# keichi/sdn-mpi-router

Measured on AMD Instinct MI355X. Metric: all-pairs routes/sec + % HBM roofline, k=48 fat-tree, 1/2/4/8 MI355X, higher is better.
Workload: dtype int32; 1 GPU; fat_tree:48 all-pairs dfs route tables (find_route); fabric=fat_tree:48, V=2880, E=110592, table_layout=packed, endpoints=host-bearing switches (host pairs), parallelism=sources sharded over 1 GPU(s), steps_in_flight=1

## Files before the change

### include/sdnroute.h

```cpp
#ifndef SDNROUTE_H
#define SDNROUTE_H

#include <stdint.h>

#ifdef __cplusplus
extern "C" {
#endif

#define SDNR_ABI_VERSION 1

#define SDNR_OK          0
#define SDNR_ERR_INVAL (-22)
#define SDNR_ERR_NOMEM (-12)
#define SDNR_ERR_NODEV (-19)
#define SDNR_ERR_STATE (-77)
#define SDNR_ERR_HIP   (-5)

#define SDNR_DEVICE_PTRS 0x1u
#define SDNR_TIMING      0x2u
#define SDNR_SAME_TABLES 0x4u
#define SDNR_LOADS_TO_ROOT 0x8u
#define SDNR_LOADS_SPLIT_HOP 0x10u
#define SDNR_LFA_LINK_ONLY 0x20u

// ... 139 lines not shown
                         double *level, int32_t max_rounds, double *used,
                         int32_t *nrounds , uint32_t flags);

int sdnr_edge_ports(sdnr_ctx *ctx, const uint64_t *ends, int32_t nends,
                    const uint64_t *ports, int32_t nports, uint8_t *is_edge,
                    uint32_t flags);

int sdnr_last_kernel_ms(sdnr_ctx *ctx, float *ms);

int sdnr_last_launches(const sdnr_ctx *ctx, int32_t *launches);

int sdnr_last_dfs_searched(sdnr_ctx *ctx, int32_t *n);

int sdnr_last_dfs_form(const sdnr_ctx *ctx, int32_t *form);

int sdnr_last_sweeps(const sdnr_ctx *ctx, int32_t *sweeps);

const char *sdnr_last_kernel(const sdnr_ctx *ctx);

#ifdef __cplusplus
}
#endif

#endif
```

### sdn-mpi-router_amd/csrc/capi.hip

```cpp
#include <stdarg.h>
#include <stdio.h>
#include <stdlib.h>
#include <string.h>

#include <algorithm>
#include <array>
#include <map>
#include <string>
#include <thread>
#include <vector>

#include "common.h"

static thread_local char g_err[512] = "";

int sdnr_fail(int code, const char *fmt, ...)
{
    va_list ap;
    va_start(ap, fmt);
    vsnprintf(g_err, sizeof g_err, fmt, ap);
    va_end(ap);
    return code;
}

// ... 142 lines not shown
    if (c->twin_rep) (void)hipFree(c->twin_rep);
    c->twin_rep = nullptr;
    c->has_twins = false;
    ++c->upload_gen;
    memset(c->live_ring, 0, sizeof c->live_ring);
    if (c->radj16 && c->radj_owned) (void)hipFree(c->radj16);
    if (c->runs) (void)hipFree(c->runs);
    c->runs = nullptr;
    c->runs_R = 0;
    if (c->adjb) (void)hipFree(c->adjb);
    if (c->adjp) (void)hipFree(c->adjp);
    if (c->radjx) (void)hipFree(c->radjx);
    c->adjb = nullptr;
    c->adjp = nullptr;
    c->radjx = nullptr;
    if (c->adj16) (void)hipFree(c->adj16);
    if (c->deg32) (void)hipFree(c->deg32);
    if (c->radjw) (void)hipFree(c->radjw);
    c->radjw = nullptr;
    if (c->radjc) (void)hipFree(c->radjc);
    c->radjc = nullptr;
    if (c->dict_bp) (void)hipFree(c->dict_bp);
    if (c->dict_bt) (void)hipFree(c->dict_bt);
    if (c->dict_off) (void)hipFree(c->dict_off);
    c->dict_bp = nullptr;
    c->dict_bt = nullptr;
    c->dict_off = nullptr;
    c->dict_P = 0;
    c->dict_NB = 0;
    c->dict_bpw = 0;
// ... 276 lines not shown
    int rc;
    if ((rc = upload(reinterpret_cast<int32_t **>(&ctx->dict_bp), bp.data(), bp.size() * 4, 0,
                     ctx->stream)) ||
        (rc = upload(reinterpret_cast<int32_t **>(&ctx->dict_bt), bt.data(), bt.size() * 4, 0,
                     ctx->stream)) ||
        (rc = upload(&ctx->dict_off, off.data(), off.size() * 4, 0, ctx->stream)))
        return rc;
    SDNR_HIP(hipStreamSynchronize(ctx->stream));
    ctx->dict_P = (int32_t)tuples.size();
    ctx->dict_NB = (int32_t)blocks.size();
    ctx->dict_bpw = bpw;
    return SDNR_OK;
}

static int upload_twins(sdnr_ctx *ctx, int32_t V, int32_t E, const int32_t *row_ptr,
                        const int32_t *col)
{
    if (V == 0) return SDNR_OK;
    std::vector<int32_t> in_ptr((size_t)V + 1, 0), in_col((size_t)E);
    for (int32_t e = 0; e < E; ++e) in_ptr[(size_t)col[e] + 1]++;
    for (int32_t v = 0; v < V; ++v) in_ptr[(size_t)v + 1] += in_ptr[v];
    {
        std::vector<int32_t> fill(in_ptr.begin(), in_ptr.end() - 1);
        for (int32_t u = 0; u < V; ++u)
            for (int32_t e = row_ptr[u]; e < row_ptr[u + 1]; ++e) in_col[fill[col[e]]++] = u;
    }
    std::vector<uint64_t> hash((size_t)V);
    std::vector<int32_t> rep((size_t)V), order;
    auto mix = [](uint64_t h, uint64_t x) {
        h ^= x + 0x9E3779B97F4A7C15ull + (h << 6) + (h >> 2);
        return h * 0xFF51AFD7ED558CCDull;
// ... 26 lines not shown
            for (size_t k = i; k < j; ++k) {
                const int32_t r = order[k];
                if (rep[r] == r && same(row_ptr, col, r, v) &&
                    same(in_ptr.data(), in_col.data(), r, v)) {
                    rep[v] = r;
                    any = true;
                    break;
                }
            }
        }
    }
    int rc = upload(&ctx->twin_rep, rep.data(), sizeof(int32_t) * (size_t)V, 0, ctx->stream);
    if (rc) return rc;
    SDNR_HIP(hipStreamSynchronize(ctx->stream));
    ctx->has_twins = any;
    return SDNR_OK;
}

int sdnr_graph_upload(sdnr_ctx *ctx, int32_t V, int32_t E, const int32_t *row_ptr,
                      const int32_t *col, const int32_t *port)
{
    CHECK_CTX(ctx);
    int rc = graph_upload_one(ctx, V, E, row_ptr, col, port);
    for (int k = 0; k < ctx->npeers && !rc; ++k)
        rc = graph_upload_one(ctx->peers[k], V, E, row_ptr, col, port);
    if (rc) return rc;
    SDNR_HIP(hipSetDevice(ctx->device));
    return SDNR_OK;
}

// ... 22 lines not shown
            if (e > a && col[e] <= col[e - 1])
                return sdnr_fail(SDNR_ERR_INVAL,
                                 "graph_upload: row %d not strictly ascending at %d", u, e);
        }
    }
    SDNR_HIP(hipSetDevice(ctx->device));
    SDNR_HIP(hipStreamSynchronize(ctx->stream));
    free_graph(ctx);
    int rc;
    if ((rc = upload(&ctx->row_ptr, row_ptr, sizeof(int32_t) * ((size_t)V + 1), 0, ctx->stream)) ||
        (rc = upload(&ctx->col, col, sizeof(int32_t) * (size_t)E, kPad, ctx->stream)) ||
        (rc = upload(&ctx->port, port, sizeof(int32_t) * (size_t)E, kPad, ctx->stream))) {
        free_graph(ctx);
        return rc;
    }
    if ((rc = upload_twins(ctx, V, E, row_ptr, col))) {
        free_graph(ctx);
        return rc;
    }
    int32_t W = 0;
    if (maxdeg > 0 && maxdeg <= SDNR_WAVE && (size_t)V * maxdeg <= 2 * (size_t)E + 64)
        W = maxdeg;
    if (const char *f = getenv("SDNROUTE_ELL"))
        if (!strcmp(f, "0")) W = 0;
    if (W > 0) {
        std::vector<int32_t> ec((size_t)V * W, -1), ep((size_t)V * W, -1);
        for (int32_t u = 0; u < V; ++u)
            for (int32_t e = row_ptr[u]; e < row_ptr[u + 1]; ++e) {
                ec[(size_t)u * W + (e - row_ptr[u])] = col[e];
                ep[(size_t)u * W + (e - row_ptr[u])] = port[e];
            }
// ... 22 lines not shown
                                        hipMemcpyHostToDevice, ctx->stream);
            }
            if (he == hipSuccess) he = hipStreamSynchronize(ctx->stream);
            if (he != hipSuccess) {
                free_graph(ctx);
                return sdnr_hip_fail(he, "graph_upload(ell16)");
            }
        }
        SDNR_HIP(hipStreamSynchronize(ctx->stream));
        if ((rc = upload_dict(ctx, V, W, row_ptr, col))) {
            free_graph(ctx);
            return rc;
        }
    }
    int32_t max_indeg = 0x7FFFFFFF;
    if (V < 65535 && maxdeg <= SDNR_WAVE) {
        const size_t rows = ((size_t)V + 1) * SDNR_WAVE;
        std::vector<uint16_t> a16(rows, (uint16_t)V), r16(rows, (uint16_t)V);
        std::vector<int32_t> indeg((size_t)V + 1, 0);
        std::vector<uint32_t> d32(((size_t)V + 2) & ~(size_t)1, 0u);
        for (int32_t u = 0; u < V; ++u) {
            const int32_t d = row_ptr[u + 1] - row_ptr[u];
            d32[(size_t)u] = (uint32_t)d;
            for (int32_t e = row_ptr[u]; e < row_ptr[u + 1]; ++e) {
                a16[(size_t)u * SDNR_WAVE + (e - row_ptr[u])] = (uint16_t)col[e];
                indeg[col[e]]++;
            }
        }
        int32_t maxin = 0;
        for (int32_t v = 0; v < V; ++v) maxin = indeg[v] > maxin ? indeg[v] : maxin;
        max_indeg = maxin;
        bool sym = true;
        if (maxin <= SDNR_WAVE) {
            std::vector<int32_t> fill((size_t)V, 0);
            for (int32_t u = 0; u < V; ++u)
                for (int32_t e = row_ptr[u]; e < row_ptr[u + 1]; ++e) {
                    const int32_t v = col[e];
                    r16[(size_t)v * SDNR_WAVE + fill[v]++] = (uint16_t)u;
                }
            sym = a16 == r16;
        }
        hipError_t he = hipMalloc(reinterpret_cast<void **>(&ctx->adj16), rows * 2);
        if (he == hipSuccess)
            he = hipMemcpyAsync(ctx->adj16, a16.data(), rows * 2, hipMemcpyHostToDevice, ctx->stream);
        if (he == hipSuccess && maxin <= SDNR_WAVE) {
            he = hipMalloc(reinterpret_cast<void **>(&ctx->deg32), d32.size() * 4);
            if (he == hipSuccess)
                he = hipMemcpyAsync(ctx->deg32, d32.data(), d32.size() * 4, hipMemcpyHostToDevice,
                                    ctx->stream);
            if (he == hipSuccess && sym) {
                ctx->radj16 = ctx->adj16;
            } else if (he == hipSuccess) {
                he = hipMalloc(reinterpret_cast<void **>(&ctx->radj16), rows * 2);
                ctx->radj_owned = he == hipSuccess;
                if (he == hipSuccess)
                    he = hipMemcpyAsync(ctx->radj16, r16.data(), rows * 2, hipMemcpyHostToDevice,
                                        ctx->stream);
            }
        }
        const size_t dummy = (((size_t)V + 1 + 31) & ~(size_t)31);
        if (he == hipSuccess && maxin <= SDNR_WAVE && dummy + SDNR_WAVE <= 0xFFFF) {
            std::vector<uint16_t> w16(r16.size());
            const std::vector<uint16_t> &src16 = sym ? a16 : r16;
            const bool pair = maxin <= SDNR_WAVE / 2;
            const char *pe = sdnr_tune_env("SDNROUTE_DFS_PAIR");
            ctx->radj_pair = pair && !(pe && !strcmp(pe, "0"));
            auto at = [&](size_t i) {
                return ctx->radj_pair ? (i & ~(size_t)(SDNR_WAVE / 2)) : i;
            };
            for (size_t i = 0; i < w16.size(); ++i) {
                const int x = src16[at(i)];
                w16[i] = (uint16_t)(x == V ? (int)(dummy + i % SDNR_WAVE) : (x ^ ((x >> 3) & 31)));
            }
            he = hipMalloc(reinterpret_cast<void **>(&ctx->radjw), w16.size() * 2);
            if (he == hipSuccess)
                he = hipMemcpyAsync(ctx->radjw, w16.data(), w16.size() * 2, hipMemcpyHostToDevice,
                                    ctx->stream);
            if (he == hipSuccess) he = hipStreamSynchronize(ctx->stream);
            const size_t dummyc = ((((size_t)V + 2) >> 1) + 31) & ~(size_t)31;
            if (he == hipSuccess && 2 * (dummyc + SDNR_WAVE) <= 0xFFFF) {
                for (size_t i = 0; i < w16.size(); ++i) {
                    const int x = src16[at(i)];
                    const int h = x >> 1;
                    w16[i] = (uint16_t)(x == V ? (int)(2 * (dummyc + i % SDNR_WAVE))
                                               : ((h ^ ((h >> 3) & 31)) << 1) | (x & 1));
                }
                he = hipMalloc(reinterpret_cast<void **>(&ctx->radjc), w16.size() * 2);
                if (he == hipSuccess)
                    he = hipMemcpyAsync(ctx->radjc, w16.data(), w16.size() * 2,
                                        hipMemcpyHostToDevice, ctx->stream);
                if (he == hipSuccess) he = hipStreamSynchronize(ctx->stream);
            }
        }
#ifdef SDNR_DIAG_VARIANTS
        const char *rf = getenv("SDNROUTE_RUNS");
        if (he == hipSuccess && maxin <= SDNR_WAVE && !(rf && !strcmp(rf, "0"))) {
            const int m = encode_runs(V, a16, 0, nullptr);
            const int R = m <= 2 ? 2 : (m <= 4 ? 4 : 0);
            if (R) {
                std::vector<uint32_t> w;
                encode_runs(V, a16, R, &w);
                he = hipMalloc(reinterpret_cast<void **>(&ctx->runs), w.size() * 4);
                if (he == hipSuccess)
                    he = hipMemcpyAsync(ctx->runs, w.data(), w.size() * 4, hipMemcpyHostToDevice,
                                        ctx->stream);
                if (he == hipSuccess) he = hipStreamSynchronize(ctx->stream);
                ctx->runs_R = R;
            }
// ... 29 lines not shown
            if (he == hipSuccess) he = hipMalloc(reinterpret_cast<void **>(&ctx->adjp), ap.size());
            if (he == hipSuccess)
                he = hipMemcpyAsync(ctx->adjp, ap.data(), ap.size(), hipMemcpyHostToDevice,
                                    ctx->stream);
            if (he == hipSuccess) he = hipMalloc(reinterpret_cast<void **>(&ctx->radjx), rx.size() * 4);
            if (he == hipSuccess)
                he = hipMemcpyAsync(ctx->radjx, rx.data(), rx.size() * 4, hipMemcpyHostToDevice,
                                    ctx->stream);
            if (he == hipSuccess) he = hipStreamSynchronize(ctx->stream);
        }
#endif
        if (he == hipSuccess) he = hipStreamSynchronize(ctx->stream);
        if (he != hipSuccess) {
            free_graph(ctx);
            return sdnr_hip_fail(he, "graph_upload(adj16)");
        }
    }
    bool symmetric = true;
    for (int32_t u = 0; u < V && symmetric; ++u)
        for (int32_t e = row_ptr[u]; e < row_ptr[u + 1]; ++e) {
            const int32_t v = col[e];
            int32_t lo = row_ptr[v], hi = row_ptr[v + 1];
            while (lo < hi) {
                const int32_t mid = (lo + hi) >> 1;
                if (col[mid] < u) lo = mid + 1; else hi = mid;
            }
            if (lo == row_ptr[v + 1] || col[lo] != u) {
                symmetric = false;
                break;
            }
// ... 1027 lines not shown
        sum += got;
    }
    SDNR_HIP(hipSetDevice(ctx->device));
    *n = sum;
    return SDNR_OK;
}

int sdnr_last_dfs_form(const sdnr_ctx *ctx, int32_t *form)
{
    CHECK_CTX(ctx);
    if (!form) return sdnr_fail(SDNR_ERR_INVAL, "sdnr_last_dfs_form: null out");
    *form = ctx->dfs_form;
    return SDNR_OK;
}

int sdnr_last_launches(const sdnr_ctx *ctx, int32_t *launches)
{
    CHECK_CTX(ctx);
    if (!launches) return sdnr_fail(SDNR_ERR_INVAL, "sdnr_last_launches: null out");
    *launches = ctx->last_launches;
    return SDNR_OK;
}

int sdnr_last_kernel_ms(sdnr_ctx *ctx, float *ms)
{
    CHECK_CTX(ctx);
    if (!ms) return sdnr_fail(SDNR_ERR_INVAL, "sdnr_last_kernel_ms: null ms");
    if (!ctx->timed) return sdnr_fail(SDNR_ERR_STATE, "sdnr_last_kernel_ms: last call untimed");
    SDNR_HIP(hipSetDevice(ctx->device));
    SDNR_HIP(hipEventSynchronize(ctx->ev1));
// ... 6 lines not shown
```

### sdn-mpi-router_amd/csrc/common.h

```cpp
#pragma once

#include <hip/hip_runtime.h>
#include <stdlib.h>
#include <stdint.h>
#include <stddef.h>

#include "../../include/sdnroute.h"

#define SDNR_WAVE 64
#define SDNR_LDS_PER_CU (160 * 1024)
#define SDNR_MAX_LDS_PER_BLOCK (160 * 1024)


__device__ __forceinline__ int lane_id() { return (int)__lane_id(); }

__device__ __forceinline__ int lanes_below(uint64_t m) {
    return (int)__builtin_amdgcn_mbcnt_hi((uint32_t)(m >> 32),
                                          __builtin_amdgcn_mbcnt_lo((uint32_t)m, 0u));
}

__device__ __forceinline__ int uniform(int x) {
    return __builtin_amdgcn_readfirstlane(x);
}

__device__ __forceinline__ int read_lane(int x, int lane) {
    return __builtin_amdgcn_readlane(x, lane);
}

__device__ __forceinline__ int highest_lane(uint64_t m) { return 63 - __clzll(m); }

__device__ __forceinline__ int lds_swz(int x) { return x ^ ((x >> 3) & 31); }


constexpr int kLiveRing = 8;

struct sdnr_ctx {
    int device = 0;
    int num_cus = 256;
    hipStream_t own_stream = nullptr;
    hipStream_t stream = nullptr;

    int32_t V = -1, E = 0, max_deg = 0;
    uint64_t deg2_sum = 0;
    int32_t max_indeg = 0x7FFFFFFF;
    int32_t W = 0;
    int32_t *row_ptr = nullptr, *col = nullptr, *port = nullptr;
    uint32_t *cost = nullptr;
    bool has_cost = false;
    int32_t *ell_col = nullptr, *ell_port = nullptr;
// ... 5 lines not shown
    int32_t dict_P = 0, dict_NB = 0, dict_bpw = 0;
    uint16_t *adj16 = nullptr;
    uint16_t *radj16 = nullptr;
    uint32_t *deg32 = nullptr;
    uint16_t *radjw = nullptr;
    uint16_t *radjc = nullptr;
    bool radj_owned = false;
    bool radj_pair = false;
    uint32_t *runs = nullptr;
    int32_t runs_R = 0;
    uint64_t *adjb = nullptr;
    uint8_t *adjp = nullptr;
    uint32_t *radjx = nullptr;
    int32_t *twin_rep = nullptr;
    bool has_twins = false;
    int32_t dfs_nsrc = 0;
    bool dfs_folded = false;
    int32_t dfs_form = 0;
    unsigned long long *h_live = nullptr;
    struct {
        uint32_t seq0, seq1, gen;
        int32_t nsrc;
    } live_ring[kLiveRing] = {};
    int live_head = 0;
    uint32_t live_seq = 0;
    uint32_t upload_gen = 0;

    void *scratch = nullptr;
    size_t scratch_bytes = 0;
    void *stage = nullptr;
// ... 206 lines not shown
```

### sdn-mpi-router_amd/csrc/dfs.hip

```cpp
#include <stdlib.h>
#include <string.h>

#include <type_traits>

#include "common.h"

namespace {

constexpr int kRing = 1024;

template <bool ELL, bool HOPS>
__global__ __launch_bounds__(64) void dfs_lds_wide_kernel(
    int V, int W, const int32_t *__restrict__ row_ptr,
    const int32_t *__restrict__ col, const int32_t *__restrict__ port,
    const int32_t *__restrict__ src, int nsrc, int32_t *__restrict__ out_parent,
    int32_t *__restrict__ out_port, int32_t *__restrict__ out_hops)
{
    extern __shared__ __attribute__((aligned(16))) uint32_t lds[];
    const int VW = (V + 31) >> 5;
    const int VWp = (VW + 3) & ~3;
    uint32_t *vis = lds;
    uint32_t *stk = vis + VWp;
    uint32_t *ps = stk + V;
    uint16_t *dep = reinterpret_cast<uint16_t *>(ps + V);
// ... 1420 lines not shown
            atomicAdd(&g_stamp[4], z_qw);
            atomicAdd(&g_stamp[5], z_push);
            atomicAdd(&g_stamp[6], z_sp);
            atomicAdd(&g_stamp[7], z_rf);
            atomicAdd(&g_stamp[8], z_rfc);
        }
#endif
    } else {
        split_writer<NS, HOPS, PK>(V, W, ell_port, qrec, qdep, ctl, lane, out_parent, out_port,
                                   out_hops, err, flags);
    }
}

__device__ __forceinline__ int swz(int x) { return lds_swz(x); }

template <int NW, bool HOPS, bool PACKED, bool C16, int PAIR, bool SPEC = false>
__global__ __launch_bounds__(NW * 64, C16 ? 7 : 1) void dfs_async_kernel(
    int V, const uint16_t *__restrict__ adj, const uint16_t *__restrict__ radj,
    const uint32_t *__restrict__ deg, const int32_t *__restrict__ row_ptr,
    const int32_t *__restrict__ port, int W, const int32_t *__restrict__ ell_port,
    const int32_t *__restrict__ src, int nsrc, int32_t *__restrict__ out_parent,
    int32_t *__restrict__ out_port, int32_t *__restrict__ out_hops, int *__restrict__ err,
    int flags, const int32_t *__restrict__ live)
{
    static_assert(NW >= 2, "wave 0 searches, the others decrement");
    if (live) nsrc = min(nsrc, *live);
    constexpr int U = 4;
    constexpr int S = NW - 1;
    constexpr int RING = 512;
#ifndef SDNR_ASYNC_G
#define SDNR_ASYNC_G 8
#endif
#ifndef SDNR_ASYNC_FLUSH_U
#define SDNR_ASYNC_FLUSH_U 6
#endif
#ifndef SDNR_ASYNC_G_DW
#define SDNR_ASYNC_G_DW 16
#endif
#ifndef SDNR_ASYNC_G_P1
#define SDNR_ASYNC_G_P1 8
// ... 29 lines not shown
            return (x >> ((v & 1) << 4)) & 0xFFFFu;
        } else {
            return __hip_atomic_load(&cnt[swz(v)], __ATOMIC_RELAXED, __HIP_MEMORY_SCOPE_WORKGROUP);
        }
    };
    uint16_t *ring = reinterpret_cast<uint16_t *>(ps + PWp + (HOPS ? ((V + 1) >> 1) : 0));
    int *ctl = reinterpret_cast<int *>(ring + RING);
    const int lane = lane_id();
    const int w = uniform((int)(threadIdx.x >> 6));
#ifdef SDNR_STAMPS
    unsigned long long kstart;
    SDNR_STAMP(kstart);
#endif

    for (int si = blockIdx.x; si < nsrc; si += gridDim.x) {
        const int s = uniform(src[si]);
        int32_t *prow = out_parent + (size_t)si * V;
        int32_t *trow = PACKED ? nullptr : out_port + (size_t)si * V;
        const size_t hb = (size_t)si * V;
        if (s < 0 || s >= V) {
            for (int v = threadIdx.x; v < V; v += blockDim.x) {
                prow[v] = -1;
                if (!PACKED) trow[v] = -1;
                if (HOPS) put_hop(out_hops, hb + v, -1, flags);
            }
            continue;
        }
#ifdef SDNR_STAMPS
        unsigned long long ph0, ph1, ph2, ph3;
        SDNR_STAMP(ph0);
#endif
        for (int i = threadIdx.x; i < VW; i += blockDim.x) vis[i] = 0u;
        if constexpr (C16) {
            const int nw = (V + 2) >> 1;
            for (int i0 = threadIdx.x; i0 < nw; i0 += U * blockDim.x) {
                uint2 dg[U];
#pragma unroll
                for (int k = 0; k < U; ++k) {
                    const int i = i0 + k * (int)blockDim.x;
                    dg[k] = reinterpret_cast<const uint2 *>(deg)[i < nw ? i : 0];
                }
// ... 14 lines not shown
#pragma unroll
                for (int k = 0; k < U; ++k) {
                    const int i = i0 + k * (int)blockDim.x;
                    if (i <= V) cnt[swz(i)] = dg[k];
                }
            }
        }
        if (threadIdx.x < 2 + S) ctl[threadIdx.x] = 0;
        __syncthreads();
#ifdef SDNR_STAMPS
        SDNR_STAMP(ph1);
#endif

        if (w == 0) {
            if (flags & kFlagPrio) __builtin_amdgcn_s_setprio(3);
            if (lane == 0) {
                vis[s >> 5] |= 1u << (s & 31);
                vis[V >> 5] |= 1u << (V & 31);
                if (C16) ps16[swz(s)] = (uint16_t)s;
                else ps[swz(s)] = (uint32_t)s;
                if (HOPS) dep[s] = 0;
                stk[0] = (uint16_t)s;
                ring[0] = (uint16_t)s;
            }
            __builtin_amdgcn_fence(__ATOMIC_RELEASE, "workgroup");
            if (lane == 0) __hip_atomic_store(&ctl[0], 1, __ATOMIC_RELAXED, __HIP_MEMORY_SCOPE_WORKGROUP);
            int pub = 1, pubd = 1, sp = 1, lo = 0;
            constexpr int NPF = 1;
            int pu[NPF];
            uint16_t xp[NPF];
#pragma unroll
            for (int k = 0; k < NPF; ++k) {
                pu[k] = -1;
                xp[k] = (uint16_t)V;
            }
#ifdef SDNR_STAMPS
            unsigned long long st_t0, st_t1, st_row = 0, st_cand = 0, st_false = 0, st_bp = 0,
                                               st_miss = 0, st_skip = 0, st_tc = 0, st_skipc = 0,
                                               st_pushc = 0;
            SDNR_STAMP(st_t0);
            st_tc = st_t0;
#endif
// ... 228 lines not shown
                        if (g < n && r[g] != V) {
                            if (C16) atomicSub(&cnt[swz(r[g] >> 1)], 1u << ((r[g] & 1) << 4));
                            else atomicSub(&cnt[swz(r[g])], 1u);
                        }
                }
                j += n * S;
                if (lane == 0) __hip_atomic_store(&ctl[2 + w - 1], j, __ATOMIC_RELAXED, __HIP_MEMORY_SCOPE_WORKGROUP);
            }
        }
        __syncthreads();
#ifdef SDNR_STAMPS
        SDNR_STAMP(ph2);
#endif

        constexpr int UF = SDNR_ASYNC_FLUSH_U;
        for (int v0 = threadIdx.x; v0 < V; v0 += UF * blockDim.x) {
            int p[UF], sl[UF], pt[UF];
#pragma unroll
            for (int k = 0; k < UF; ++k) {
                const int v = v0 + k * (int)blockDim.x;
                p[k] = -1;
                sl[k] = -1;
                if (v < V && ((vis[v >> 5] >> (v & 31)) & 1u)) {
                    if (C16) {
                        p[k] = (int)ps16[swz(v)];
                        if (v != s) sl[k] = (int)sl8[swz(v)];
                    } else {
                        const uint32_t xx = ps[swz(v)];
                        p[k] = (int)(xx & 0xFFFFu);
                        if (v != s) sl[k] = (int)(xx >> 16);
// ... 449 lines not shown
    else
        hipLaunchKernelGGL(dfs_pack_kernel, dim3(ctx->num_cus * 8), dim3(256), 0, ctx->stream,
                           n, parent, port, tree);
    SDNR_HIP(hipGetLastError());
    return SDNR_OK;
}

#ifdef SDNR_DIAG_VARIANTS
static bool dfs_bits_default(const char *force)
{
    return force && !strcmp(force, "bits");
}

#endif

template <int N_, bool H_, bool P_, bool SPEC>
static auto async_pick(bool c16, bool pair, bool dw)
{
    return c16 ? (pair ? dfs_async_kernel<N_, H_, P_, true, 1>
                       : dfs_async_kernel<N_, H_, P_, true, 0>)
               : (pair ? dfs_async_kernel<N_, H_, P_, false, 1>
                       : (dw ? dfs_async_kernel<N_, H_, P_, false, 2>
                             : dfs_async_kernel<N_, H_, P_, false, 0, SPEC>));
}

__global__ __launch_bounds__(256) void dfs_hops16_kernel(size_t n, const int32_t *__restrict__ h,
                                                         uint16_t *__restrict__ out)
{
    for (size_t i = blockIdx.x * (size_t)blockDim.x + threadIdx.x; i < n;
         i += (size_t)gridDim.x * blockDim.x)
        out[i] = (uint16_t)h[i];
}

static bool dfs_small(const sdnr_ctx *ctx, int nsrc)
{
    const int V = ctx->V;
    const size_t small_b = dfs_lds_bytes_small(V);
    const size_t cu_blocks_small = SDNR_LDS_PER_CU / small_b;
// ... 10 lines not shown
    return small;
}

static bool dfs_count_ok(const sdnr_ctx *ctx, bool hops)
{
    return ctx->adj16 != nullptr && ctx->radj16 != nullptr && ctx->V < 65535 &&
           dfs_lds_bytes_count(ctx->V, hops) <= SDNR_MAX_LDS_PER_BLOCK;
}

static bool dfs_async(const sdnr_ctx *ctx, int nsrc, bool hops)
{
    const char *force = getenv("SDNROUTE_DFS_STRATEGY");
    return dfs_count_ok(ctx, hops) &&
           dfs_lds_bytes_async(ctx->V, hops) <= SDNR_MAX_LDS_PER_BLOCK &&
           (force ? !strcmp(force, "async") : dfs_small(ctx, nsrc));
}

#ifndef SDNR_FOLD_LOW_FORM
#define SDNR_FOLD_LOW_FORM 2
#endif

static int dfs_dispatch(sdnr_ctx *ctx, const int32_t *d_src, int32_t nsrc,
                        int32_t *d_parent, int32_t *d_port, int32_t *d_hops, uint32_t *d_tree,
                        bool slots = false, bool hops16 = false,
                        const int32_t *d_live = nullptr, bool low = false, int32_t live_n = 0)
{
    const int V = ctx->V;
    if (nsrc == 0 || V == 0) return SDNR_OK;
    const bool packed = d_tree != nullptr;
    const bool ell = ctx->W > 0;
// ... 80 lines not shown
    const bool coop = !count && coop_ok && (force ? !strcmp(force, "coop") : small);
    if (async) {
        int *err = ctx->d_err;
        auto per_cu = [&](int w, bool c) {
            size_t b = SDNR_LDS_PER_CU / dfs_lds_bytes_async(V, hops, c);
            if (b > (size_t)(32 / w)) b = 32 / w;
            return b < 1 ? (size_t)1 : b;
        };
        auto compact = [&](int w) {
            bool c = per_cu(w, true) > per_cu(w, false) &&
                     (size_t)ctx->num_cus * per_cu(w, false) < (size_t)nsrc;
            if (const char *f = getenv("SDNROUTE_DFS_C16")) c = !strcmp(f, "1");
            return c;
        };
        const char *pz = getenv("SDNROUTE_DFS_PRESWZ");
        auto rows_of = [&](bool c) { return c ? ctx->radjc : ctx->radjw; };
        auto preswz_of = [&](bool c) { return rows_of(c) && !(pz && !strcmp(pz, "0")); };
        int nw = dfs_async_waves(ctx, nsrc);
        if (low && d_live && live_n > 0) {
            const int cw = dfs_async_waves(ctx, live_n);
            const bool cc = compact(cw);
            if (!cc && !(preswz_of(cc) && ctx->radj_pair)) nw = cw;
        }
        const bool c16 = compact(nw);
        const size_t cl = dfs_lds_bytes_async(V, hops, c16);
        const size_t cpc = per_cu(nw, c16);
        const uint16_t *rw = rows_of(c16);
        const bool preswz = preswz_of(c16);
        bool specpop = true;
        if (const char *f = getenv("SDNROUTE_DFS_SPECPOP")) specpop = !strcmp(f, "1");
        bool spec = specpop;
// ... 5 lines not shown
        if (dq) dw = preswz && !pair && !c16 && !strcmp(dq, "1");
        if (low && d_live && !c16 && !pair) {
            if (SDNR_FOLD_LOW_FORM & 1) spec = false;
            if (SDNR_FOLD_LOW_FORM & 2) dw = preswz;
            ctx->dfs_form = kDfsFormLow;
        }
        int cgrid = (int)((size_t)ctx->num_cus * cpc);
        if (cgrid > nsrc) cgrid = nsrc;
        static const char *names[] = {"", "", "dfs_async_kernel<2>", "dfs_async_kernel<3>",
                                      "dfs_async_kernel<4>", "dfs_async_kernel<5>",
                                      "dfs_async_kernel<6>", "", "dfs_async_kernel<8>"};
        ctx->last_kernel = names[nw];
#define SDNR_ASYNC_P(N_, H_, P_)                                                             \
    do {                                                                                     \
        constexpr bool kSpecOk = N_ == 4;                    \
        auto k = spec && kSpecOk ? async_pick<N_, H_, P_, kSpecOk>(c16, pair, dw)            \
                                 : async_pick<N_, H_, P_, false>(c16, pair, dw);             \
        allow_full_lds(k);                                                                   \
        hipLaunchKernelGGL(k, dim3(cgrid), dim3(N_ * 64), cl, ctx->stream, V, ctx->adj16,    \
                           preswz ? rw : ctx->radj16, ctx->deg32, ctx->row_ptr,              \
                           ctx->port, ctx->W, ctx->ell_port, d_src, nsrc,                    \
                           P_ ? reinterpret_cast<int32_t *>(d_tree) : d_parent, d_port,      \
                           d_hops, err, aflags, d_live);                                     \
    } while (0)
#define SDNR_ASYNC(N_, H_) SDNR_ASYNC_P(N_, H_, false)
        if (packed) {
            static const char *pnames[] = {"", "", "dfs_async_kernel<2,packed>",
                                           "dfs_async_kernel<3,packed>",
                                           "dfs_async_kernel<4,packed>",
                                           "dfs_async_kernel<5,packed>",
                                           "dfs_async_kernel<6,packed>", "",
                                           "dfs_async_kernel<8,packed>"};
            ctx->last_kernel = pnames[nw];
            if (hops) {
                static const char *hnames[] = {"", "", "", "dfs_async_kernel<3,packed,hops>",
                                               "dfs_async_kernel<4,packed,hops>", "",
                                               "dfs_async_kernel<6,packed,hops>"};
                const int hw = nw <= 3 ? 3 : (nw >= 6 ? 6 : 4);
// ... 509 lines not shown
                return false;
            *count = (int32_t)(uint32_t)w;
            return true;
        }
    return false;
}

int sdnr_launch_dfs(sdnr_ctx *ctx, const int32_t *d_src, int32_t nsrc,
                    int32_t *d_parent, int32_t *d_port, int32_t *d_hops, uint32_t *d_tree,
                    bool slots, bool hops16)
{
    const int V = ctx->V;
    ctx->dfs_nsrc = nsrc;
    ctx->dfs_folded = false;
    ctx->dfs_form = kDfsFormFull;
    if (nsrc == 0 || V == 0 || !dfs_fold(ctx, nsrc))
        return dfs_dispatch(ctx, d_src, nsrc, d_parent, d_port, d_hops, d_tree, slots, hops16);
    const bool packed = d_tree != nullptr;
    const size_t n = (size_t)nsrc * (size_t)V;
    const int hbytes = d_hops ? (hops16 ? 2 : 4) : 0;
    auto up = [](size_t x) { return (x + 255) & ~(size_t)255; };
    const size_t o_csrc = 256, o_lead = o_csrc + up(4 * (size_t)nsrc),
                 o_lsrc = o_lead + up(4 * (size_t)nsrc), o_tab = o_lsrc + up(4 * (size_t)nsrc),
                 o_t0 = o_tab + up(8 * (size_t)V), o_t1 = o_t0 + up(4 * n),
                 o_h = o_t1 + (packed ? 0 : up(4 * n)), need = o_h + up((size_t)hbytes * n);
    if (need > kFoldScratchBytes)
        return dfs_dispatch(ctx, d_src, nsrc, d_parent, d_port, d_hops, d_tree, slots, hops16);
    int rc = sdnr_reserve(&ctx->scratch3, &ctx->scratch3_bytes, need);
    if (rc) return rc;
    char *sb = static_cast<char *>(ctx->scratch3);
// ... 63 lines not shown
```

### sdn-mpi-router_amd/sdnmpi_amd/_native.py

```python

import ctypes
import os
import threading

import numpy as np

__all__ = ["NativeUnavailable", "SdnrError", "library", "library_path",
           "Context", "DEVICE_PTRS", "TIMING", "UNREACHED", "DIST_INF", "TREE_NONE",
           "EXPORTED_SYMBOLS", "unpack_tree"]

_HERE = os.path.dirname(os.path.abspath(__file__))
_LIB_NAME = "libsdnroute.so"

DEVICE_PTRS = 0x1
TIMING = 0x2
SAME_TABLES = 0x4
LOADS_TO_ROOT = 0x8
LOADS_SPLIT_HOP = 0x10
LFA_LINK_ONLY = 0x20
UNREACHED = -1
DIST_INF = 0xFFFF
TREE_NONE = 0xFFFFFFFF
COST_INF = 0xFFFFFFFF
UTIL_MAX = 0xFFFFFFFE
# ... 1 lines not shown
TREE_PORT16 = 1
TREE_SLOT = 2
ABI_VERSION = 1

EXPORTED_SYMBOLS = (
    "sdnr_abi_version", "sdnr_build_id", "sdnr_last_error", "sdnr_device_count", "sdnr_create",
    "sdnr_create_multi", "sdnr_device_list", "sdnr_destroy", "sdnr_set_stream", "sdnr_synchronize", "sdnr_graph_upload",
    "sdnr_graph_info", "sdnr_dfs_tables", "sdnr_dfs_tables_packed", "sdnr_dfs_tables_slots",
    "sdnr_dfs_tables_tree", "sdnr_tree_pack", "sdnr_shortest_tables", "sdnr_route_expand_packed",
    "sdnr_apsp", "sdnr_route_offsets", "sdnr_route_expand", "sdnr_ecmp_counts",
    "sdnr_ecmp_routes",
    "sdnr_last_kernel_ms", "sdnr_last_kernel", "sdnr_last_launches", "sdnr_last_sweeps",
    "sdnr_edge_ports", "sdnr_dfs_rows_affected", "sdnr_link_loads",
    "sdnr_ecmp_link_loads", "sdnr_graph_costs", "sdnr_cost_tables",
    "sdnr_cost_ecmp_link_loads", "sdnr_graph_twin_reps", "sdnr_last_dfs_searched",
    "sdnr_last_dfs_form",
    "sdnr_failure_ecmp_link_loads", "sdnr_lfa_tables", "sdnr_whatif_ecmp_link_loads",
    "sdnr_widest_tables", "sdnr_fair_rates", "sdnr_ecmp_fair_rates",
)


class NativeUnavailable(RuntimeError):
    """libsdnroute.so could not be loaded (not built, or no HIP runtime)."""


class SdnrError(RuntimeError):
    def __init__(self, code, msg):
        super(SdnrError, self).__init__("sdnroute error %d: %s" % (code, msg))
        self.code = code


# ... 45 lines not shown
        "sdnr_cost_tables": ([vp, vp, i32, vp, vp, vp, u32], c_int),
        "sdnr_cost_ecmp_link_loads": ([vp, vp, i32, vp, vp, vp, vp, u32], c_int),
        "sdnr_failure_ecmp_link_loads": ([vp, vp, i32, vp, vp, vp, i32, vp, vp, vp, vp, vp, u32],
                                         c_int),
        "sdnr_lfa_tables": ([vp, vp, vp, i32, vp, vp, vp, vp, u32], c_int),
        "sdnr_whatif_ecmp_link_loads": ([vp, vp, i32, vp, vp, vp, i32, vp, vp, vp, vp, vp, vp, vp,
                                         vp, vp, u32], c_int),
        "sdnr_widest_tables": ([vp, vp, vp, vp, i32, vp, vp, vp, u32], c_int),
        "sdnr_fair_rates": ([vp, vp, i32, i32, vp, vp, vp, vp, vp, i32, vp, vp, vp, vp, i32, vp,
                             ctypes.POINTER(i32), u32], c_int),
        "sdnr_ecmp_fair_rates": ([vp, vp, i32, vp, vp, vp, vp, vp, i32, vp, vp, vp, vp, i32, vp,
                                  ctypes.POINTER(i32), u32], c_int),
        "sdnr_graph_twin_reps": ([vp, vp], c_int),
        "sdnr_last_dfs_searched": ([vp, ctypes.POINTER(i32)], c_int),
        "sdnr_last_dfs_form": ([vp, ctypes.POINTER(i32)], c_int),
    }
    older_ok = "SDNROUTE_LIB" in os.environ
    for name, (args, res) in sig.items():
        if older_ok and not hasattr(L, name):
            continue
        f = getattr(L, name)
        f.argtypes = args
        f.restype = res
    return L


def library():
    global _lib
    with _lock:
        if _lib is not None:
# ... 468 lines not shown
    def twin_reps(self):
        rep = np.empty(max(self.V, 0), np.int32)
        _check(self._lib.sdnr_graph_twin_reps(self._h, _ptr(rep)))
        return rep

    def last_dfs_searched(self):
        n = ctypes.c_int32()
        _check(self._lib.sdnr_last_dfs_searched(self._h, ctypes.byref(n)))
        return n.value

    def last_dfs_form(self):
        n = ctypes.c_int32()
        _check(self._lib.sdnr_last_dfs_form(self._h, ctypes.byref(n)))
        return "low" if n.value else "full"

    def last_sweeps(self):
        n = ctypes.c_int32()
        _check(self._lib.sdnr_last_sweeps(self._h, ctypes.byref(n)))
        return n.value

    def last_kernel_ms(self):
        ms = ctypes.c_float()
        _check(self._lib.sdnr_last_kernel_ms(self._h, ctypes.byref(ms)))
        return ms.value
```

Measured before the change: 14140 billion routes/s.

## Run async DFS on twin-quotient graph and expand tables per vertex

Builds a quotient graph that collapses twin vertices (same neighbourhoods) into classes, with per-class adjacency, slot maps and port offsets uploaded to the device. The async DFS kernel searches the smaller quotient graph, then expands parent and port entries back to every original vertex through the class and slot lookup tables. This is meant to cut search work and LDS traffic on fat-trees, where many switches are twins. It is enabled automatically when the quotient has at most half the edges. The cost is extra indirections in the output write loop and more graph-upload memory.

```diff
diff --git a/include/sdnroute.h b/include/sdnroute.h
--- a/include/sdnroute.h
+++ b/include/sdnroute.h
@@ -177,6 +177,8 @@
 
 int sdnr_last_dfs_form(const sdnr_ctx *ctx, int32_t *form);
 
+int sdnr_last_dfs_quotient(const sdnr_ctx *ctx, int32_t *on);
+
 int sdnr_last_sweeps(const sdnr_ctx *ctx, int32_t *sweeps);
 
 const char *sdnr_last_kernel(const sdnr_ctx *ctx);
diff --git a/sdn-mpi-router_amd/csrc/capi.hip b/sdn-mpi-router_amd/csrc/capi.hip
--- a/sdn-mpi-router_amd/csrc/capi.hip
+++ b/sdn-mpi-router_amd/csrc/capi.hip
@@ -180,6 +180,21 @@
     c->adjb = nullptr;
     c->adjp = nullptr;
     c->radjx = nullptr;
+    if (c->q_radj16 && c->q_radj_owned) (void)hipFree(c->q_radj16);
+    {
+        void **qb[] = {reinterpret_cast<void **>(&c->q_adj16), reinterpret_cast<void **>(&c->q_deg32),
+                       reinterpret_cast<void **>(&c->q_radjw), reinterpret_cast<void **>(&c->q_radjc),
+                       reinterpret_cast<void **>(&c->q_cid), reinterpret_cast<void **>(&c->q_info),
+                       reinterpret_cast<void **>(&c->q_loff), reinterpret_cast<void **>(&c->q_slot),
+                       reinterpret_cast<void **>(&c->q_tab)};
+        for (void **b : qb) {
+            if (*b) (void)hipFree(*b);
+            *b = nullptr;
+        }
+    }
+    c->q_radj16 = nullptr;
+    c->q_radj_owned = false;
+    c->q_V = c->q_E = 0;
     if (c->adj16) (void)hipFree(c->adj16);
     if (c->deg32) (void)hipFree(c->deg32);
     if (c->radjw) (void)hipFree(c->radjw);
@@ -486,7 +501,7 @@
 }
 
 static int upload_twins(sdnr_ctx *ctx, int32_t V, int32_t E, const int32_t *row_ptr,
-                        const int32_t *col)
+                        const int32_t *col, std::vector<int32_t> *rep_out)
 {
     if (V == 0) return SDNR_OK;
     std::vector<int32_t> in_ptr((size_t)V + 1, 0), in_col((size_t)E);
@@ -543,6 +558,7 @@
     if (rc) return rc;
     SDNR_HIP(hipStreamSynchronize(ctx->stream));
     ctx->has_twins = any;
+    rep_out->swap(rep);
     return SDNR_OK;
 }
 
@@ -595,7 +611,8 @@
         free_graph(ctx);
         return rc;
     }
-    if ((rc = upload_twins(ctx, V, E, row_ptr, col))) {
+    std::vector<int32_t> twin_rep;
+    if ((rc = upload_twins(ctx, V, E, row_ptr, col, &twin_rep))) {
         free_graph(ctx);
         return rc;
     }
@@ -648,9 +665,17 @@
         }
     }
     int32_t max_indeg = 0x7FFFFFFF;
-    if (V < 65535 && maxdeg <= SDNR_WAVE) {
+    struct U16Rows {
+        uint16_t *adj16 = nullptr, *radj16 = nullptr, *radjw = nullptr, *radjc = nullptr;
+        uint32_t *deg32 = nullptr;
+        bool radj_owned = false, radj_pair = false;
+    };
+    auto upload_u16_rows = [ctx](U16Rows &o, int32_t V, const int32_t *row_ptr, const int32_t *col,
+                                 std::vector<uint16_t> &a16, std::vector<uint16_t> &r16, bool &sym,
+                                 int32_t &maxin, int paired) -> hipError_t {
         const size_t rows = ((size_t)V + 1) * SDNR_WAVE;
-        std::vector<uint16_t> a16(rows, (uint16_t)V), r16(rows, (uint16_t)V);
+        a16.assign(rows, (uint16_t)V);
+        r16.assign(rows, (uint16_t)V);
         std::vector<int32_t> indeg((size_t)V + 1, 0);
         std::vector<uint32_t> d32(((size_t)V + 2) & ~(size_t)1, 0u);
         for (int32_t u = 0; u < V; ++u) {
@@ -661,10 +686,9 @@
                 indeg[col[e]]++;
             }
         }
-        int32_t maxin = 0;
+        maxin = 0;
         for (int32_t v = 0; v < V; ++v) maxin = indeg[v] > maxin ? indeg[v] : maxin;
-        max_indeg = maxin;
-        bool sym = true;
+        sym = true;
         if (maxin <= SDNR_WAVE) {
             std::vector<int32_t> fill((size_t)V, 0);
             for (int32_t u = 0; u < V; ++u)
@@ -674,21 +698,21 @@
                 }
             sym = a16 == r16;
         }
-        hipError_t he = hipMalloc(reinterpret_cast<void **>(&ctx->adj16), rows * 2);
+        hipError_t he = hipMalloc(reinterpret_cast<void **>(&o.adj16), rows * 2);
         if (he == hipSuccess)
-            he = hipMemcpyAsync(ctx->adj16, a16.data(), rows * 2, hipMemcpyHostToDevice, ctx->stream);
+            he = hipMemcpyAsync(o.adj16, a16.data(), rows * 2, hipMemcpyHostToDevice, ctx->stream);
         if (he == hipSuccess && maxin <= SDNR_WAVE) {
-            he = hipMalloc(reinterpret_cast<void **>(&ctx->deg32), d32.size() * 4);
+            he = hipMalloc(reinterpret_cast<void **>(&o.deg32), d32.size() * 4);
             if (he == hipSuccess)
-                he = hipMemcpyAsync(ctx->deg32, d32.data(), d32.size() * 4, hipMemcpyHostToDevice,
+                he = hipMemcpyAsync(o.deg32, d32.data(), d32.size() * 4, hipMemcpyHostToDevice,
                                     ctx->stream);
             if (he == hipSuccess && sym) {
-                ctx->radj16 = ctx->adj16;
+                o.radj16 = o.adj16;
             } else if (he == hipSuccess) {
-                he = hipMalloc(reinterpret_cast<void **>(&ctx->radj16), rows * 2);
-                ctx->radj_owned = he == hipSuccess;
+                he = hipMalloc(reinterpret_cast<void **>(&o.radj16), rows * 2);
+                o.radj_owned = he == hipSuccess;
                 if (he == hipSuccess)
-                    he = hipMemcpyAsync(ctx->radj16, r16.data(), rows * 2, hipMemcpyHostToDevice,
+                    he = hipMemcpyAsync(o.radj16, r16.data(), rows * 2, hipMemcpyHostToDevice,
                                         ctx->stream);
             }
         }
@@ -698,17 +722,17 @@
             const std::vector<uint16_t> &src16 = sym ? a16 : r16;
             const bool pair = maxin <= SDNR_WAVE / 2;
             const char *pe = sdnr_tune_env("SDNROUTE_DFS_PAIR");
-            ctx->radj_pair = pair && !(pe && !strcmp(pe, "0"));
+            o.radj_pair = pair && (paired < 0 ? !(pe && !strcmp(pe, "0")) : paired == 1);
             auto at = [&](size_t i) {
-                return ctx->radj_pair ? (i & ~(size_t)(SDNR_WAVE / 2)) : i;
+                return o.radj_pair ? (i & ~(size_t)(SDNR_WAVE / 2)) : i;
             };
             for (size_t i = 0; i < w16.size(); ++i) {
                 const int x = src16[at(i)];
                 w16[i] = (uint16_t)(x == V ? (int)(dummy + i % SDNR_WAVE) : (x ^ ((x >> 3) & 31)));
             }
-            he = hipMalloc(reinterpret_cast<void **>(&ctx->radjw), w16.size() * 2);
+            he = hipMalloc(reinterpret_cast<void **>(&o.radjw), w16.size() * 2);
             if (he == hipSuccess)
-                he = hipMemcpyAsync(ctx->radjw, w16.data(), w16.size() * 2, hipMemcpyHostToDevice,
+                he = hipMemcpyAsync(o.radjw, w16.data(), w16.size() * 2, hipMemcpyHostToDevice,
                                     ctx->stream);
             if (he == hipSuccess) he = hipStreamSynchronize(ctx->stream);
             const size_t dummyc = ((((size_t)V + 2) >> 1) + 31) & ~(size_t)31;
@@ -719,13 +743,30 @@
                     w16[i] = (uint16_t)(x == V ? (int)(2 * (dummyc + i % SDNR_WAVE))
                                                : ((h ^ ((h >> 3) & 31)) << 1) | (x & 1));
                 }
-                he = hipMalloc(reinterpret_cast<void **>(&ctx->radjc), w16.size() * 2);
+                he = hipMalloc(reinterpret_cast<void **>(&o.radjc), w16.size() * 2);
                 if (he == hipSuccess)
-                    he = hipMemcpyAsync(ctx->radjc, w16.data(), w16.size() * 2,
+                    he = hipMemcpyAsync(o.radjc, w16.data(), w16.size() * 2,
                                         hipMemcpyHostToDevice, ctx->stream);
                 if (he == hipSuccess) he = hipStreamSynchronize(ctx->stream);
             }
         }
+        if (he == hipSuccess) he = hipStreamSynchronize(ctx->stream);
+        return he;
+    };
+    if (V < 65535 && maxdeg <= SDNR_WAVE) {
+        std::vector<uint16_t> a16, r16;
+        bool sym = true;
+        int32_t maxin = 0;
+        U16Rows o;
+        hipError_t he = upload_u16_rows(o, V, row_ptr, col, a16, r16, sym, maxin, -1);
+        ctx->adj16 = o.adj16;
+        ctx->radj16 = o.radj16;
+        ctx->deg32 = o.deg32;
+        ctx->radjw = o.radjw;
+        ctx->radjc = o.radjc;
+        ctx->radj_owned = o.radj_owned;
+        ctx->radj_pair = o.radj_pair;
+        max_indeg = maxin;
 #ifdef SDNR_DIAG_VARIANTS
         const char *rf = getenv("SDNROUTE_RUNS");
         if (he == hipSuccess && maxin <= SDNR_WAVE && !(rf && !strcmp(rf, "0"))) {
@@ -785,6 +826,84 @@
         if (he != hipSuccess) {
             free_graph(ctx);
             return sdnr_hip_fail(he, "graph_upload(adj16)");
+        }
+        if (ctx->has_twins && ctx->radj16) {
+            std::vector<int32_t> cmax_of((size_t)V), id_of((size_t)V, -1);
+            for (int32_t v = 0; v < V; ++v) cmax_of[twin_rep[v]] = v;
+            int32_t Vq = 0;
+            for (int32_t v = 0; v < V; ++v)
+                if (cmax_of[twin_rep[v]] == v) id_of[twin_rep[v]] = Vq++;
+            std::vector<uint32_t> cidrk((size_t)V + kPad, 0u), info((size_t)Vq + 1, 0u),
+                csize((size_t)Vq, 0u);
+            for (int32_t v = 0; v < V; ++v) {
+                const uint32_t c = (uint32_t)id_of[twin_rep[v]];
+                cidrk[v] = c | (csize[c]++ << 16);
+                info[c] = (uint32_t)v;
+            }
+            for (int32_t c = 0; c < Vq; ++c) info[c] |= csize[c] > 1 ? 1u << 16 : 0u;
+            std::vector<int32_t> qptr((size_t)Vq + 1, 0), qcol, tmp;
+            std::vector<uint32_t> loff((size_t)Vq * SDNR_WAVE + kPad, 0u);
+            std::vector<uint8_t> mslot;
+            for (int32_t c = 0; c < Vq; ++c) {
+                const int32_t P = (int32_t)(info[c] & 0xFFFFu);
+                tmp.clear();
+                for (int32_t e = row_ptr[P]; e < row_ptr[P + 1]; ++e)
+                    tmp.push_back((int32_t)(cidrk[col[e]] & 0xFFFFu));
+                std::sort(tmp.begin(), tmp.end());
+                tmp.erase(std::unique(tmp.begin(), tmp.end()), tmp.end());
+                for (size_t j = 0; j < tmp.size(); ++j) {
+                    loff[(size_t)c * SDNR_WAVE + j] = (uint32_t)mslot.size();
+                    mslot.resize(mslot.size() + csize[tmp[j]], 0);
+                }
+                for (int32_t e = row_ptr[P]; e < row_ptr[P + 1]; ++e) {
+                    const uint32_t ck = cidrk[col[e]];
+                    const size_t j = (size_t)(std::lower_bound(tmp.begin(), tmp.end(),
+                                                               (int32_t)(ck & 0xFFFFu)) - tmp.begin());
+                    mslot[loff[(size_t)c * SDNR_WAVE + j] + (ck >> 16)] = (uint8_t)(e - row_ptr[P]);
+                }
+                qcol.insert(qcol.end(), tmp.begin(), tmp.end());
+                qptr[(size_t)c + 1] = (int32_t)qcol.size();
+            }
+            mslot.resize(mslot.size() + kPad, 0);
+            qcol.push_back(0);
+            std::vector<uint16_t> qa16, qr16;
+            bool qsym = true;
+            int32_t qmaxin = 0;
+            U16Rows q;
+            he = upload_u16_rows(q, Vq, qptr.data(), qcol.data(), qa16, qr16, qsym, qmaxin,
+                                 ctx->radj_pair ? 1 : 0);
+            ctx->q_adj16 = q.adj16;
+            ctx->q_radj16 = q.radj16;
+            ctx->q_deg32 = q.deg32;
+            ctx->q_radjw = q.radjw;
+            ctx->q_radjc = q.radjc;
+            ctx->q_radj_owned = q.radj_owned;
+            auto put = [&](void **dst, const void *src, size_t bytes) {
+                if (he == hipSuccess) he = hipMalloc(dst, bytes);
+                if (he == hipSuccess)
+                    he = hipMemcpyAsync(*dst, src, bytes, hipMemcpyHostToDevice, ctx->stream);
+            };
+            put(reinterpret_cast<void **>(&ctx->q_cid), cidrk.data(), cidrk.size() * 4);
+            put(reinterpret_cast<void **>(&ctx->q_info), info.data(), info.size() * 4);
+            put(reinterpret_cast<void **>(&ctx->q_loff), loff.data(), loff.size() * 4);
+            put(reinterpret_cast<void **>(&ctx->q_slot), mslot.data(), mslot.size());
+            const sdnr_quot qt{V, ctx->q_cid, ctx->q_info, ctx->q_loff, ctx->q_slot};
+            put(reinterpret_cast<void **>(&ctx->q_tab), &qt, sizeof qt);
+            if (he == hipSuccess) he = hipStreamSynchronize(ctx->stream);
+            if (he != hipSuccess) {
+                free_graph(ctx);
+                return sdnr_hip_fail(he, "graph_upload(quotient)");
+            }
+            if (!ctx->radjw && ctx->q_radjw) {
+                (void)hipFree(ctx->q_radjw);
+                ctx->q_radjw = nullptr;
+            }
+            if (!ctx->radjc && ctx->q_radjc) {
+                (void)hipFree(ctx->q_radjc);
+                ctx->q_radjc = nullptr;
+            }
+            ctx->q_V = Vq;
+            ctx->q_E = qptr[(size_t)Vq];
         }
     }
     bool symmetric = true;
@@ -1842,6 +1961,14 @@
     return SDNR_OK;
 }
 
+int sdnr_last_dfs_quotient(const sdnr_ctx *ctx, int32_t *on)
+{
+    CHECK_CTX(ctx);
+    if (!on) return sdnr_fail(SDNR_ERR_INVAL, "sdnr_last_dfs_quotient: null out");
+    *on = ctx->dfs_quotient ? 1 : 0;
+    return SDNR_OK;
+}
+
 int sdnr_last_launches(const sdnr_ctx *ctx, int32_t *launches)
 {
     CHECK_CTX(ctx);
diff --git a/sdn-mpi-router_amd/csrc/common.h b/sdn-mpi-router_amd/csrc/common.h
--- a/sdn-mpi-router_amd/csrc/common.h
+++ b/sdn-mpi-router_amd/csrc/common.h
@@ -33,6 +33,12 @@
 
 
 constexpr int kLiveRing = 8;
+
+struct sdnr_quot {
+    int32_t VR;
+    const uint32_t *cid, *info, *loff;
+    const uint8_t *slot;
+};
 
 struct sdnr_ctx {
     int device = 0;
@@ -68,6 +74,14 @@
     uint32_t *radjx = nullptr;
     int32_t *twin_rep = nullptr;
     bool has_twins = false;
+    int32_t q_V = 0, q_E = 0;
+    uint16_t *q_adj16 = nullptr, *q_radj16 = nullptr, *q_radjw = nullptr, *q_radjc = nullptr;
+    uint32_t *q_deg32 = nullptr;
+    bool q_radj_owned = false;
+    uint32_t *q_cid = nullptr, *q_info = nullptr, *q_loff = nullptr;
+    uint8_t *q_slot = nullptr;
+    struct sdnr_quot *q_tab = nullptr;
+    bool dfs_quotient = false;
     int32_t dfs_nsrc = 0;
     bool dfs_folded = false;
     int32_t dfs_form = 0;
diff --git a/sdn-mpi-router_amd/csrc/dfs.hip b/sdn-mpi-router_amd/csrc/dfs.hip
--- a/sdn-mpi-router_amd/csrc/dfs.hip
+++ b/sdn-mpi-router_amd/csrc/dfs.hip
@@ -1458,16 +1458,19 @@
 
 __device__ __forceinline__ int swz(int x) { return lds_swz(x); }
 
-template <int NW, bool HOPS, bool PACKED, bool C16, int PAIR, bool SPEC = false>
+template <int NW, bool HOPS, bool PACKED, bool C16, int PAIR, bool SPEC = false, bool QUOT = false>
 __global__ __launch_bounds__(NW * 64, C16 ? 7 : 1) void dfs_async_kernel(
     int V, const uint16_t *__restrict__ adj, const uint16_t *__restrict__ radj,
     const uint32_t *__restrict__ deg, const int32_t *__restrict__ row_ptr,
     const int32_t *__restrict__ port, int W, const int32_t *__restrict__ ell_port,
     const int32_t *__restrict__ src, int nsrc, int32_t *__restrict__ out_parent,
     int32_t *__restrict__ out_port, int32_t *__restrict__ out_hops, int *__restrict__ err,
-    int flags, const int32_t *__restrict__ live)
+    int flags, const int32_t *__restrict__ live,
+    const sdnr_quot *__restrict__ qt)
 {
     static_assert(NW >= 2, "wave 0 searches, the others decrement");
+    constexpr bool quot = QUOT;
+    const int VT = quot ? uniform((int)qt->VR) : V;
     if (live) nsrc = min(nsrc, *live);
     constexpr int U = 4;
     constexpr int S = NW - 1;
@@ -1527,17 +1530,23 @@
 #endif
 
     for (int si = blockIdx.x; si < nsrc; si += gridDim.x) {
-        const int s = uniform(src[si]);
-        int32_t *prow = out_parent + (size_t)si * V;
-        int32_t *trow = PACKED ? nullptr : out_port + (size_t)si * V;
-        const size_t hb = (size_t)si * V;
-        if (s < 0 || s >= V) {
-            for (int v = threadIdx.x; v < V; v += blockDim.x) {
+        const int sr = uniform(src[si]);
+        int32_t *prow = out_parent + (size_t)si * VT;
+        int32_t *trow = PACKED ? nullptr : out_port + (size_t)si * VT;
+        const size_t hb = (size_t)si * VT;
+        if (sr < 0 || sr >= VT) {
+            for (int v = threadIdx.x; v < VT; v += blockDim.x) {
                 prow[v] = -1;
                 if (!PACKED) trow[v] = -1;
                 if (HOPS) put_hop(out_hops, hb + v, -1, flags);
             }
             continue;
+        }
+        int s = sr;
+        bool rootvis = true;
+        if constexpr (quot) {
+            s = uniform((int)(qt->cid[sr] & 0xFFFFu));
+            rootvis = uniform((int)(qt->info[s] >> 16)) == 0;
         }
 #ifdef SDNR_STAMPS
         unsigned long long ph0, ph1, ph2, ph3;
@@ -1582,8 +1591,9 @@
 
         if (w == 0) {
             if (flags & kFlagPrio) __builtin_amdgcn_s_setprio(3);
+            const int pub0 = rootvis ? 1 : 0;
             if (lane == 0) {
-                vis[s >> 5] |= 1u << (s & 31);
+                if (rootvis) vis[s >> 5] |= 1u << (s & 31);
                 vis[V >> 5] |= 1u << (V & 31);
                 if (C16) ps16[swz(s)] = (uint16_t)s;
                 else ps[swz(s)] = (uint32_t)s;
@@ -1592,8 +1602,8 @@
                 ring[0] = (uint16_t)s;
             }
             __builtin_amdgcn_fence(__ATOMIC_RELEASE, "workgroup");
-            if (lane == 0) __hip_atomic_store(&ctl[0], 1, __ATOMIC_RELAXED, __HIP_MEMORY_SCOPE_WORKGROUP);
-            int pub = 1, pubd = 1, sp = 1, lo = 0;
+            if (lane == 0) __hip_atomic_store(&ctl[0], pub0, __ATOMIC_RELAXED, __HIP_MEMORY_SCOPE_WORKGROUP);
+            int pub = pub0, pubd = pub0, sp = 1, lo = 0;
             constexpr int NPF = 1;
             int pu[NPF];
             uint16_t xp[NPF];
@@ -1852,6 +1862,70 @@
 #endif
 
         constexpr int UF = SDNR_ASYNC_FLUSH_U;
+        if constexpr (quot) {
+            const uint32_t *__restrict__ qcid = qt->cid, *__restrict__ qinfo = qt->info,
+                                         *__restrict__ qloff = qt->loff;
+            const uint8_t *__restrict__ qslot = qt->slot;
+            for (int v0 = threadIdx.x; v0 < VT; v0 += UF * blockDim.x) {
+                uint32_t ck[UF], lf[UF];
+                int p[UF], sl[UF], pt[UF];
+#pragma unroll
+                for (int k = 0; k < UF; ++k) {
+                    const int v = v0 + k * (int)blockDim.x;
+                    ck[k] = qcid[v < VT ? v : 0];
+                }
+#pragma unroll
+                for (int k = 0; k < UF; ++k) {
+                    const int v = v0 + k * (int)blockDim.x;
+                    const int c = (int)(ck[k] & 0xFFFFu);
+                    p[k] = -1;
+                    sl[k] = -1;
+                    lf[k] = 0;
+                    if (v < VT && v == sr) {
+                        p[k] = sr;
+                    } else if (v < VT && ((vis[c >> 5] >> (c & 31)) & 1u)) {
+                        int pc, qs;
+                        if (C16) {
+                            pc = (int)ps16[swz(c)];
+                            qs = (int)sl8[swz(c)];
+                        } else {
+                            const uint32_t xx = ps[swz(c)];
+                            pc = (int)(xx & 0xFFFFu);
+                            qs = (int)(xx >> 16);
+                        }
+                        p[k] = pc == s ? sr : (int)(qinfo[pc] & 0xFFFFu);
+                        lf[k] = qloff[(size_t)pc * 64 + qs];
+                        sl[k] = 0;
+                    }
+                }
+#pragma unroll
+                for (int k = 0; k < UF; ++k)
+                    if (sl[k] >= 0) sl[k] = (int)qslot[lf[k] + (ck[k] >> 16)];
+#pragma unroll
+                for (int k = 0; k < UF; ++k) {
+                    pt[k] = -1;
+                    if (sl[k] >= 0)
+                        pt[k] = W > 0 ? ell_port[(size_t)p[k] * W + sl[k]]
+                                      : port[row_ptr[p[k]] + sl[k]];
+                }
+#pragma unroll
+                for (int k = 0; k < UF; ++k) {
+                    const int v = v0 + k * (int)blockDim.x;
+                    if (v < VT) {
+                        if (PACKED) {
+                            prow[v] = (int32_t)(((uint32_t)p[k] & 0xFFFFu) |
+                                                ((uint32_t)pt[k] << 16));
+                        } else {
+                            prow[v] = p[k];
+                            trow[v] = pt[k];
+                        }
+                        if (HOPS)
+                            put_hop(out_hops, hb + v,
+                                    p[k] < 0 ? -1 : (v == sr ? 0 : (int)dep[ck[k] & 0xFFFFu]), flags);
+                    }
+                }
+            }
+        } else
         for (int v0 = threadIdx.x; v0 < V; v0 += UF * blockDim.x) {
             int p[UF], sl[UF], pt[UF];
 #pragma unroll
@@ -2331,14 +2405,14 @@
 
 #endif
 
-template <int N_, bool H_, bool P_, bool SPEC>
+template <int N_, bool H_, bool P_, bool SPEC, bool Q_ = false>
 static auto async_pick(bool c16, bool pair, bool dw)
 {
-    return c16 ? (pair ? dfs_async_kernel<N_, H_, P_, true, 1>
-                       : dfs_async_kernel<N_, H_, P_, true, 0>)
-               : (pair ? dfs_async_kernel<N_, H_, P_, false, 1>
-                       : (dw ? dfs_async_kernel<N_, H_, P_, false, 2>
-                             : dfs_async_kernel<N_, H_, P_, false, 0, SPEC>));
+    return c16 ? (pair ? dfs_async_kernel<N_, H_, P_, true, 1, false, Q_>
+                       : dfs_async_kernel<N_, H_, P_, true, 0, false, Q_>)
+               : (pair ? dfs_async_kernel<N_, H_, P_, false, 1, false, Q_>
+                       : (dw ? dfs_async_kernel<N_, H_, P_, false, 2, false, Q_>
+                             : dfs_async_kernel<N_, H_, P_, false, 0, SPEC, Q_>));
 }
 
 __global__ __launch_bounds__(256) void dfs_hops16_kernel(size_t n, const int32_t *__restrict__ h,
@@ -2379,6 +2453,16 @@
     return dfs_count_ok(ctx, hops) &&
            dfs_lds_bytes_async(ctx->V, hops) <= SDNR_MAX_LDS_PER_BLOCK &&
            (force ? !strcmp(force, "async") : dfs_small(ctx, nsrc));
+}
+
+static bool dfs_quotient(const sdnr_ctx *ctx)
+{
+    if (!ctx->q_tab || ctx->q_V <= 0) return false;
+    if (const char *f = getenv("SDNROUTE_DFS_QUOTIENT")) {
+        if (!strcmp(f, "0")) return false;
+        if (!strcmp(f, "1")) return true;
+    }
+    return 2 * (int64_t)ctx->q_E <= (int64_t)ctx->E;
 }
 
 #ifndef SDNR_FOLD_LOW_FORM
@@ -2489,7 +2573,11 @@
             return c;
         };
         const char *pz = getenv("SDNROUTE_DFS_PRESWZ");
-        auto rows_of = [&](bool c) { return c ? ctx->radjc : ctx->radjw; };
+        const bool quot = dfs_quotient(ctx);
+        ctx->dfs_quotient = quot;
+        auto rows_of = [&](bool c) {
+            return quot ? (c ? ctx->q_radjc : ctx->q_radjw) : (c ? ctx->radjc : ctx->radjw);
+        };
         auto preswz_of = [&](bool c) { return rows_of(c) && !(pz && !strcmp(pz, "0")); };
         int nw = dfs_async_waves(ctx, nsrc);
         if (low && d_live && live_n > 0) {
@@ -2525,14 +2613,19 @@
 #define SDNR_ASYNC_P(N_, H_, P_)                                                             \
     do {                                                                                     \
         constexpr bool kSpecOk = N_ == 4;                    \
-        auto k = spec && kSpecOk ? async_pick<N_, H_, P_, kSpecOk>(c16, pair, dw)            \
-                                 : async_pick<N_, H_, P_, false>(c16, pair, dw);             \
+        auto k = quot ? (spec && kSpecOk ? async_pick<N_, H_, P_, kSpecOk, true>(c16, pair, dw) \
+                                         : async_pick<N_, H_, P_, false, true>(c16, pair, dw)) \
+                      : (spec && kSpecOk ? async_pick<N_, H_, P_, kSpecOk>(c16, pair, dw)    \
+                                         : async_pick<N_, H_, P_, false>(c16, pair, dw));    \
         allow_full_lds(k);                                                                   \
-        hipLaunchKernelGGL(k, dim3(cgrid), dim3(N_ * 64), cl, ctx->stream, V, ctx->adj16,    \
-                           preswz ? rw : ctx->radj16, ctx->deg32, ctx->row_ptr,              \
+        hipLaunchKernelGGL(k, dim3(cgrid), dim3(N_ * 64), cl, ctx->stream,                   \
+                           quot ? ctx->q_V : V, quot ? ctx->q_adj16 : ctx->adj16,            \
+                           preswz ? rw : (quot ? ctx->q_radj16 : ctx->radj16),               \
+                           quot ? ctx->q_deg32 : ctx->deg32, ctx->row_ptr,                   \
                            ctx->port, ctx->W, ctx->ell_port, d_src, nsrc,                    \
                            P_ ? reinterpret_cast<int32_t *>(d_tree) : d_parent, d_port,      \
-                           d_hops, err, aflags, d_live);                                     \
+                           d_hops, err, aflags, d_live,                                      \
+                           quot ? ctx->q_tab : static_cast<const sdnr_quot *>(nullptr));     \
     } while (0)
 #define SDNR_ASYNC(N_, H_) SDNR_ASYNC_P(N_, H_, false)
         if (packed) {
@@ -3072,6 +3165,7 @@
     ctx->dfs_nsrc = nsrc;
     ctx->dfs_folded = false;
     ctx->dfs_form = kDfsFormFull;
+    ctx->dfs_quotient = false;
     if (nsrc == 0 || V == 0 || !dfs_fold(ctx, nsrc))
         return dfs_dispatch(ctx, d_src, nsrc, d_parent, d_port, d_hops, d_tree, slots, hops16);
     const bool packed = d_tree != nullptr;
diff --git a/sdn-mpi-router_amd/sdnmpi_amd/_native.py b/sdn-mpi-router_amd/sdnmpi_amd/_native.py
--- a/sdn-mpi-router_amd/sdnmpi_amd/_native.py
+++ b/sdn-mpi-router_amd/sdnmpi_amd/_native.py
@@ -39,7 +39,7 @@
     "sdnr_edge_ports", "sdnr_dfs_rows_affected", "sdnr_link_loads",
     "sdnr_ecmp_link_loads", "sdnr_graph_costs", "sdnr_cost_tables",
     "sdnr_cost_ecmp_link_loads", "sdnr_graph_twin_reps", "sdnr_last_dfs_searched",
-    "sdnr_last_dfs_form",
+    "sdnr_last_dfs_form", "sdnr_last_dfs_quotient",
     "sdnr_failure_ecmp_link_loads", "sdnr_lfa_tables", "sdnr_whatif_ecmp_link_loads",
     "sdnr_widest_tables", "sdnr_fair_rates", "sdnr_ecmp_fair_rates",
 )
@@ -115,6 +115,7 @@
         "sdnr_graph_twin_reps": ([vp, vp], c_int),
         "sdnr_last_dfs_searched": ([vp, ctypes.POINTER(i32)], c_int),
         "sdnr_last_dfs_form": ([vp, ctypes.POINTER(i32)], c_int),
+        "sdnr_last_dfs_quotient": ([vp, ctypes.POINTER(i32)], c_int),
     }
     older_ok = "SDNROUTE_LIB" in os.environ
     for name, (args, res) in sig.items():
@@ -613,6 +614,11 @@
         _check(self._lib.sdnr_last_dfs_form(self._h, ctypes.byref(n)))
         return "low" if n.value else "full"
 
+    def last_dfs_quotient(self):
+        n = ctypes.c_int32()
+        _check(self._lib.sdnr_last_dfs_quotient(self._h, ctypes.byref(n)))
+        return n.value
+
     def last_sweeps(self):
         n = ctypes.c_int32()
         _check(self._lib.sdnr_last_sweeps(self._h, ctypes.byref(n)))
```

Result: faster. 14680 billion routes/s (median of 6 runs) (+3.8%).
